# InfiniteNightmare/HNSW-Slim

Measured on AMD Instinct MI355X. Metric: QPS @ recall@10>=0.95 (SIFT-1M d=128, k=10), higher is better.
Workload: dtype f32

## Files before the change

hnsw-slim_amd/csrc/capi_search.cpp:

```cpp
#include "capi_internal.hpp"

#include <cstdio>

static constexpr size_t kMaxLaunchQueries = 32768;

static PlanInput plan_input(const hs_index *ix, size_t k, size_t nq, int mode, bool has_filter, bool want_raw) {
  PlanInput in{};
  const DevIndex &d = ix->dev;
  in.n = ix->info.n; in.dim = ix->info.dim;
  in.has_tile0 = d.tile0 != nullptr; in.has_uptile = d.uptile != nullptr;
  in.maxlevel = d.maxlevel; in.threshold_level = d.threshold_level; in.has_deleted = d.has_deleted; in.kind = d.kind;
  in.ef = ix->ef; in.k = k; in.nq = nq; in.mode = mode;
  in.user_cand_cap = ix->user_cand_cap; in.user_hash_slots = ix->user_hash_slots; in.grow_cand = ix->grow_cand; in.grow_hash = ix->grow_hash;
  in.exact_order = ix->exact_order; in.want_raw = want_raw; in.has_filter = has_filter;
  in.row_fmt = ix->row_fmt; in.f32_resident = ix->f32_resident;
  in.diag = diag();
  return in;
}

static hs_status search_dev_group(hs_index *ix, const float *d_q, size_t nq, size_t k, int mode, uint32_t *l32,
                                  uint64_t *l64, float *dd, uint32_t *cnt, uint32_t *stats, Pair *raw, uint32_t *rawsz,
                                  hipStream_t stream, bool first_group, size_t nq_total, const FilterUse *fu = nullptr) {
  if (!ix) return fail(HS_ERR_INVALID, "null index");
  if (k == 0) return fail(HS_ERR_INVALID, "k must be > 0");
  if (mode != HS_MODE_SLIM_IDS && mode != HS_MODE_PQ) return fail(HS_ERR_INVALID, "bad mode");
  if (ix->info.kind == HS_KIND_SLIMQ) return fail(HS_ERR_INVALID, "SlimQ index: use hs_slimq_search_batch");
  if (mode == HS_MODE_SLIM_IDS && ix->info.kind != HS_KIND_SLIM)
    return fail(HS_ERR_INVALID, "HS_MODE_SLIM_IDS needs a Slim index (searchKnn(q,k,tableint*) exists on HierarchicalNSWSlim only)");
  if (nq > 0x7FFFFFFFu) return fail(HS_ERR_INVALID, "nq too large");
  if (nq == 0) return HS_OK;
  SearchPlan p;
  const char *why = "";
  hs_status ps = plan_search(plan_input(ix, k, nq, mode, fu != nullptr, raw != nullptr), p, &why);
  if (ps != HS_OK) return fail(ps, why);
  HIP_TRY(hipSetDevice(ix->device));
  hs_index::StreamWs *w = ix->stream_ws(stream);
  HIP_TRY(w->status.ensure(nq));
  HIP_TRY(w->spill.ensure(nq * (size_t)p.spill_stride));
  if (w->counters.n < 48) {
    HIP_TRY(w->counters.ensure(48));
    HIP_TRY(hipMemsetAsync(w->counters.p, 0, 48 * sizeof(uint32_t), stream));
  }
  if (first_group) w->last_nq += nq_total;
  if (p.split) {
    HIP_TRY(w->entry.ensure(nq * 4));
    HIP_TRY(w->order.ensure(nq));
  }
  HIP_TRY(w->fb.ensure((size_t)kFbGrid * ((size_t)kFbCand * 2 + kFbSpill)));
  ix->last_kernel = p.name;

  SearchArgs a{};
  FilterArgs fa{};
  if (fu) fa = FilterArgs{fu->fs->bits.p, fu->d_of_query, w->counters.p + 12, (uint32_t)fu->fs->row_words, (uint32_t)fu->fs->nf};
  const FilterArgs *fap = fu ? &fa : nullptr;
  a.queries = d_q; a.nq = (uint32_t)nq; a.k = (uint32_t)k; a.ef = p.ef;
  a.mode = mode; a.mark_ep = (int32_t)p.mark_ep;
  a.out_labels32 = l32; a.out_labels64 = l64; a.out_dists = dd; a.out_counts = cnt; a.stats = stats;
  a.raw_top = raw; a.raw_size = rawsz; a.raw_stride = p.ef;
  a.status = w->status.p;
  a.spill = w->spill.p; a.spill_slots = kSpillSlots; a.spill_stride = p.spill_stride; a.cand2_cap = kCand2Cap;
  a.log_cap = p.log_cap; a.hop_cap = p.hop_cap;
  a.flat = p.flat;
  a.cand_cap = p.cand_cap; a.hash_slots = p.hash_slots; a.vis_bits = p.vis_bits; a.hash_fill_shift = p.hash_fill_shift;
  if (p.family == HS_PLAN_FLAT) { a.fl_nb = p.fl_nb; a.fl_mul = p.fl_mul; a.fl_sh = p.fl_sh; }
  a.counters = w->counters.p; a.pass_id = 0;
  a.select_mask = 1u << ST_TODO; a.grid = (uint32_t)nq;
  auto strict_go = [&](int rows) {
    return rows != ROWS_F32 ? launch_strict_narrow(ix->dev, a, ix->narrow.p, rows, stream, fap) : launch_strict(ix->dev, a, stream, fap);
  };
  auto pass0 = [&]() {
    switch (p.family) {
      case HS_PLAN_FLAT: return p.rows != ROWS_F32 ? launch_flatk_narrow(ix->dev, a, ix->narrow.p, p.rows, stream) : launch_flatk(ix->dev, a, stream);
      case HS_PLAN_LEAN: return launch_lean(ix->dev, a, stream);
      case HS_PLAN_FAST: return p.rows != ROWS_F32 ? launch_fast_narrow(ix->dev, a, ix->narrow.p, p.rows, stream, fap) : launch_fast(ix->dev, a, stream, fap);
      default: return strict_go(p.rows);
    }
  };
  if (p.split) {
    a.entry = reinterpret_cast<uint4 *>(w->entry.p); a.order = w->order.p;
    a.phase = 1;
    HIP_TRY(pass0());
    if (p.skip_order) a.order = nullptr;
    else HIP_TRY(launch_order(a.entry, w->order.p, (uint32_t)nq, stream));
    a.phase = 2;
    HIP_TRY(pass0());
    a.phase = 0;
  } else {
    HIP_TRY(pass0());
  }
  a.select_mask = p.rerun_select_mask; a.grid = (uint32_t)std::min<size_t>(nq, kFbGrid);
  a.cand_cap = p.rerun_cand_cap; a.hash_slots = p.rerun_hash_slots; a.vis_bits = 0; a.hash_fill_shift = 0;
  a.fb_cand = w->fb.p; a.fb_spill = w->fb.p + (size_t)kFbGrid * kFbCand * 2; a.spill_slots = kFbSpill;
  a.counters = w->counters.p + 8; a.pass_id = 2;
  HIP_TRY(strict_go(p.rerun_rows));
  return HS_OK;
}

hs_status search_dev(hs_index *ix, const float *d_q, size_t nq, size_t k, int mode, uint32_t *l32, uint64_t *l64, float *dd,
                     uint32_t *cnt, uint32_t *stats, Pair *raw, uint32_t *rawsz, hipStream_t stream, const FilterUse *fu) {
  if (!ix) return fail(HS_ERR_INVALID, "null index");
  if (nq > 0x7FFFFFFFu) return fail(HS_ERR_INVALID, "nq too large");
  const size_t dim = ix->info.dim, ef = std::max(ix->ef, k);
  for (size_t off = 0; off < nq || off == 0; off += kMaxLaunchQueries) {
    const size_t m = std::min(kMaxLaunchQueries, nq - off);
    const FilterUse g{fu ? fu->fs : nullptr, fu ? fu->d_of_query + off : nullptr};
    hs_status s = search_dev_group(ix, d_q + off * dim, m, k, mode, l32 ? l32 + off * k : nullptr, l64 ? l64 + off * k : nullptr,
                                   dd ? dd + off * k : nullptr, cnt ? cnt + off : nullptr, stats ? stats + off * 4 : nullptr,
                                   raw ? raw + off * ef : nullptr, rawsz ? rawsz + off : nullptr, stream, off == 0, nq, fu ? &g : nullptr);
    if (s != HS_OK || nq == 0) return s;
  }
  return HS_OK;
}

hs_status hs_search_check(hs_index *ix, void *stream) {
  if (!ix) return fail(HS_ERR_INVALID, "null index");
  uint32_t c[13];
  HIP_TRY(hipSetDevice(ix->device));
  hs_index::StreamWs *w = ix->stream_ws((hipStream_t)stream);
  if (!w->counters.p) return HS_OK;
  HIP_TRY(hipMemcpyAsync(c, w->counters.p, sizeof(c), hipMemcpyDeviceToHost, (hipStream_t)stream));
  HIP_TRY(hipMemsetAsync(w->counters.p, 0, sizeof(c), (hipStream_t)stream));
  HIP_TRY(hipStreamSynchronize((hipStream_t)stream));
  const size_t nq = std::max<size_t>(w->last_nq, 1);
  w->last_nq = 0;
  if (diag().verbose) fprintf(stderr, "[hs check] nq %zu: visited overflow %u, candidate overflow %u, tie replays %u, visited-set spills %u | pass 2: %u %u | grow_hash %u grow_cand %u\n",
                       nq, c[0], c[1], c[2], c[3], c[8], c[9], ix->grow_hash, ix->grow_cand);
  if ((size_t)c[3] * 10 > nq && ix->grow_hash < 8 && !ix->user_hash_slots) ix->grow_hash++;
  if ((size_t)(c[1] + c[5]) * 100 > nq && ix->grow_cand < 4 && !ix->user_cand_cap) ix->grow_cand++;
  if (c[12] > 0)
    return fail(HS_ERR_INVALID, std::to_string(c[12]) + " queries named a filter index outside the filter set (count 0 returned for them)");
  if (ix->info.kind == HS_KIND_SLIMQ) {
    if (c[8] > 0) return fail(HS_ERR_CAPACITY, std::to_string(c[8]) + " queries expanded more nodes than the 64 KiB on-chip set holds");
    return HS_OK;
  }
  if (c[8] + c[9] > 0)
    return fail(HS_ERR_CAPACITY, std::to_string(c[8] + c[9]) + " queries exhausted even a whole CU's on-chip scratch");
  return HS_OK;
}

hs_status hs_debug_search_plan(const hs_plan_in *in, hs_plan_out *out) {
  if (!in || !out) return fail(HS_ERR_INVALID, "null argument");
  const char *why = "";
  hs_status s = plan_search(*in, *out, &why);
  return s == HS_OK ? s : fail(s, why);
}
hs_status hs_debug_plan_input(const hs_index *ix, size_t k, size_t nq, int has_filter, int want_raw, hs_plan_in *in) {
  if (!ix || !in) return fail(HS_ERR_INVALID, "null argument");
  *in = plan_input(ix, k, nq, HS_MODE_PQ, has_filter != 0, want_raw != 0);
  return HS_OK;
}

hs_status hs_debug_heap_ops(const uint32_t *ops, size_t n_ops, int wave_pop, uint32_t lds_slots, uint32_t *out_heap, uint32_t *out_pops,
                            uint32_t *out_n) {
  if (!ops || !out_heap || !out_pops || !out_n) return fail(HS_ERR_INVALID, "null argument");
  if (lds_slots < 2 || lds_slots > 8192 || (lds_slots & 1)) return fail(HS_ERR_INVALID, "lds_slots: even, 2..8192");
  DevBuf<uint32_t> d_ops, d_n;
  DevBuf<uint2> d_spill, d_heap, d_pops;
  HIP_TRY(d_ops.alloc(std::max<size_t>(3 * n_ops, 1)));
  HIP_TRY(d_n.alloc(2));
  HIP_TRY(d_spill.alloc(n_ops + 2));
  HIP_TRY(d_heap.alloc(n_ops + 2));
  HIP_TRY(d_pops.alloc(n_ops + 2));
  HIP_TRY(hipMemcpy(d_ops.p, ops, 3 * n_ops * sizeof(uint32_t), hipMemcpyHostToDevice));
  HIP_TRY(flat_heap_ops(d_ops.p, (uint32_t)n_ops, d_spill.p, d_heap.p, d_pops.p, d_n.p, wave_pop, lds_slots, nullptr));
// ... 162 lines not shown
```

hnsw-slim_amd/csrc/engine.hpp:

```cpp
#pragma once
#include <hip/hip_runtime.h>

#include <cstdint>

#include "heap_emul.hpp"

namespace hs {

struct DevIndex {
  const float *vec;
  const uint32_t *row_ptr0;
  const uint32_t *cols;
  const uint32_t *up_base;
  const uint32_t *up_ptr;
  const uint32_t *tile0;
  const uint2 *uptile;
  const uint64_t *labels;
  const uint8_t *deleted;
  uint32_t n, dim, tile_stride, up_stride, ep_base;
  int32_t maxlevel, threshold_level;
  uint32_t enterpoint;
  int32_t has_deleted, kind, metric;
};

enum : uint32_t { ST_TODO = 0, ST_DONE = 1, ST_OVERFLOW = 2, ST_HAZARD = 3 };

struct SearchArgs {
  const float *queries;
  uint32_t nq, k, ef;
  uint32_t cand_cap;
  uint32_t hash_slots;
  uint32_t *spill;
  uint32_t spill_slots, spill_stride, cand2_cap, log_cap;
  int32_t mode;
  int32_t mark_ep;
  uint32_t select_mask;
  uint32_t grid;
  uint32_t *out_labels32;
  uint64_t *out_labels64;
  float *out_dists;
  uint32_t *out_counts;
  uint32_t *stats;
  Pair *raw_top;
  uint32_t *raw_size;
  uint32_t raw_stride;
  uint32_t *status;
  uint32_t *counters;
  uint32_t pass_id;
  uint32_t hash_fill_shift;
  uint32_t flat;
  uint32_t hop_cap;
  uint32_t vis_bits;
  uint32_t phase;
  uint4 *entry;
  const uint32_t *order;
  void *fb_cand;
  uint32_t *fb_spill;
  uint32_t fl_nb, fl_mul, fl_sh;
};

struct FilterArgs {
  const uint32_t *rows;
  const uint32_t *of_query;
  uint32_t *bad;
  uint32_t stride, nf;
};

size_t strict_lds_bytes(uint32_t dim, uint32_t ef, uint32_t cand_cap, uint32_t hash_slots);
size_t fast_lds_bytes(uint32_t dim, uint32_t ef, uint32_t cand_cap, uint32_t hash_slots);
bool fast_supported(const DevIndex &ix, uint32_t ef, uint32_t k, bool has_filter = false);

hipError_t launch_strict(const DevIndex &ix, const SearchArgs &a, hipStream_t stream, const FilterArgs *f = nullptr);
hipError_t launch_order(const uint4 *entry, uint32_t *order, uint32_t nq, hipStream_t stream);
bool lean_supported(const DevIndex &ix, uint32_t ef, uint32_t k);
size_t lean_lds_bytes(uint32_t dim, uint32_t ef, uint32_t cand_cap, uint32_t hash_slots);
hipError_t launch_lean(const DevIndex &ix, const SearchArgs &a, hipStream_t stream);
bool flatk_supported(const DevIndex &ix, uint32_t ef, uint32_t k);
size_t flatk_lds_bytes(uint32_t dim, uint32_t ef, uint32_t nb);
uint32_t flatk_waves_per_cu(uint32_t dim, uint32_t ef);
hipError_t launch_flatk(const DevIndex &ix, const SearchArgs &a, hipStream_t stream);
hipError_t flat_heap_ops(const uint32_t *d_ops, uint32_t n_ops, uint2 *d_spill, uint2 *d_heap, uint2 *d_pops, uint32_t *d_n, int wave_pop,
                         uint32_t lds_slots, hipStream_t stream);
hipError_t launch_fast(const DevIndex &ix, const SearchArgs &a, hipStream_t stream, const FilterArgs *f = nullptr);
hipError_t launch_flatk_narrow(const DevIndex &ix, const SearchArgs &a, const void *rows, int fmt, hipStream_t stream);
hipError_t launch_strict_narrow(const DevIndex &ix, const SearchArgs &a, const void *rows, int fmt, hipStream_t stream, const FilterArgs *f = nullptr);
hipError_t launch_fast_narrow(const DevIndex &ix, const SearchArgs &a, const void *rows, int fmt, hipStream_t stream, const FilterArgs *f = nullptr);
hipError_t launch_narrow_convert(const float *d_vec, void *d_out, int fmt, uint32_t row0, uint32_t nrows, uint32_t dim, uint32_t *d_first_bad,
                                 hipStream_t stream);
hipError_t launch_narrow_widen(const void *d_rows, float *d_vec, int fmt, uint32_t row0, uint32_t nrows, uint32_t dim, hipStream_t stream);
hipError_t launch_filter_pack(const uint8_t *d_allowed, uint32_t *d_words, uint32_t n, uint32_t count, uint32_t row_words, hipStream_t stream);
hipError_t launch_filter_unpack(const uint32_t *d_row, uint8_t *d_allowed, uint32_t n, hipStream_t stream);

}
```

hnsw-slim_amd/csrc/flat_search.hip:

```cpp
#include <hip/hip_runtime.h>

#include <algorithm>
#include <cfloat>
#include <climits>

#include "dist_recipe.hpp"
#include "engine.hpp"
#include "heap_emul.hpp"
#include "narrow_load.hpp"
#include "search_common.hpp"
#include "sorted_insert.hpp"
#include "wave_util.hpp"

namespace hs {

typedef __attribute__((address_space(3))) unsigned char lds_u8;
typedef __attribute__((address_space(3))) uint32_t lds_u32;
typedef __attribute__((address_space(3))) unsigned short lds_u16;
typedef uint32_t hs_u4 __attribute__((ext_vector_type(4)));
typedef __attribute__((address_space(3))) hs_u4 lds_u128;
typedef __attribute__((address_space(3))) float lds_f32;
typedef __attribute__((address_space(3))) hs_f2 lds_f2;
typedef unsigned short hs_us2 __attribute__((ext_vector_type(2)));

static constexpr uint32_t kFlatOvfCap = 64;
static constexpr uint32_t kFlatBucketTags = 7;

struct FlatLds { uint32_t off_q, off_vis, off_ovf, off_nid, total; };
__host__ __device__ inline FlatLds flat_layout(uint32_t dim, uint32_t ef, uint32_t nb) {
  FlatLds l;
  l.off_q = 0;
  l.off_vis = align_up(dim * 4, 16);
  const uint32_t vis_bytes = nb * 16 > (ef + 1) * 8 ? nb * 16 : (ef + 1) * 8;
  l.off_ovf = l.off_vis + align_up(vis_bytes, 16);
  l.off_nid = l.off_ovf + kFlatOvfCap * 4;
  l.total = l.off_nid + 64 * 4;
  return l;
}

__device__ __forceinline__ uint32_t pk_min_u16(uint32_t a, uint32_t b) {
  return __builtin_bit_cast(uint32_t, __builtin_elementwise_min(__builtin_bit_cast(hs_us2, a), __builtin_bit_cast(hs_us2, b)));
}
template <int METRIC>
__device__ __forceinline__ int dkey(float d) {
  const int b = (int)__float_as_uint(d);
  return METRIC == METRIC_L2 ? b : (b ^ ((b >> 31) & 0x7FFFFFFF));
}
template <int METRIC>
__device__ __forceinline__ float key_dist(int k) {
  return __uint_as_float((uint32_t)(METRIC == METRIC_L2 ? k : (k ^ ((k >> 31) & 0x7FFFFFFF))));
}
static constexpr int kFKeyInf = 0x7F800000;
static constexpr uint32_t kFDone = 0x80000000u;

__device__ __forceinline__ int wave_min_i32_f(int v) {
#define HS_SHR_MINI(ctrl) v = min(v, __builtin_amdgcn_update_dpp(INT_MAX, v, ctrl, 0xf, 0xf, false))
  HS_SHR_MINI(0x111); HS_SHR_MINI(0x112); HS_SHR_MINI(0x114); HS_SHR_MINI(0x118);
#undef HS_SHR_MINI
  const int r0 = __builtin_amdgcn_readlane(v, 15), r1 = __builtin_amdgcn_readlane(v, 31);
  const int r2 = __builtin_amdgcn_readlane(v, 47), r3 = __builtin_amdgcn_readlane(v, 63);
  return min(min(r0, r1), min(r2, r3));
}

__host__ __device__ constexpr int flat_row_buffer(int d16) {
#ifdef HS_FLAT_LONG_B
  return d16 <= 0 ? 1 : d16 <= 8 ? d16 : (d16 < HS_FLAT_LONG_B ? d16 : HS_FLAT_LONG_B);
#else
  return d16 <= 0 ? 1 : d16 <= 8 ? d16 : d16 % 30 == 0 ? 30 : d16 % 32 == 0 ? 32 : d16 % 24 == 0 ? 24 : 16;
#endif
}
__host__ __device__ constexpr int flat_waves(int s, int d16) {
#ifdef HS_FLAT_WAVES
  return HS_FLAT_WAVES;
#else
#ifdef HS_FLAT_LONG_WAVES
  return d16 > 8 ? HS_FLAT_LONG_WAVES : d16 < 0 ? 3 : s > 4 ? 4 : 5;
#else
  return d16 > 8 ? 2 : d16 < 0 ? 3 : s > 4 ? 4 : 5;
#endif
#endif
}


template <int METRIC, int D16, typename ROW>
__device__ __forceinline__ float flat_dist8(const ROW *vec, uint32_t dim, const lds_u8 *qv, uint32_t rowid, int s) {
  const lds_f2 *qq = reinterpret_cast<const lds_f2 *>(qv) + s;
  hs_f2 acc = {0.f, 0.f};
  auto step = [&](const hs_f2 q2, const hs_f2 x) {
    if (METRIC == METRIC_L2) {
      const hs_f2 t = q2 - x;
      const hs_f2 p = t * t;
      acc = acc + p;
    } else {
      acc = __builtin_elementwise_fma(q2, x, acc);
    }
  };
  if constexpr (RowKind<ROW>::narrow) {
    const ROW *chunk = vec + (size_t)rowid * dim + (uint32_t)s * (dim >> 3);
    if constexpr (D16 > 0) {
      constexpr int NDW = D16 * (int)sizeof(ROW) / 2;
      static_assert(D16 * sizeof(ROW) % 2 == 0, "a lane's chunk is a whole number of dwords");
      const uint32_t *cp = reinterpret_cast<const uint32_t *>(chunk);
      uint32_t dw[NDW];
#pragma unroll
      for (int j = 0; j + 4 <= NDW; j += 4) {
        const hs_u4_a4 v = *reinterpret_cast<const hs_u4_a4 *>(cp + j);
        dw[j] = v.x; dw[j + 1] = v.y; dw[j + 2] = v.z; dw[j + 3] = v.w;
      }
      if constexpr ((NDW & 2) != 0) {
        const hs_u2_a4 v = *reinterpret_cast<const hs_u2_a4 *>(cp + (NDW & ~3));
        dw[NDW & ~3] = v.x; dw[(NDW & ~3) + 1] = v.y;
      }
      if constexpr ((NDW & 1) != 0) dw[NDW - 1] = cp[NDW - 1];
#pragma unroll
      for (int i = 0; i < D16; i++) {
        if (D16 > 8 && i % 8 == 0) __builtin_amdgcn_sched_barrier(0);
        step(qq[i * 8], narrow_pair((const ROW *)nullptr, dw, i));
      }
    } else {
      constexpr uint32_t RB = D16 == 0 ? 8u : 16u;
      const uint32_t steps = dim >> 4;
      for (uint32_t r0 = 0; r0 < steps; r0 += RB) {
        const uint32_t nb = min(RB, steps - r0);
        hs_f2 buf[RB];
#pragma unroll
        for (uint32_t i = 0; i < RB; i++)
          if (i < nb) buf[i] = narrow_pair_at(chunk, r0 + i);
#pragma unroll
        for (uint32_t i = 0; i < RB; i++)
          if (i < nb) step(qq[(r0 + i) * 8], buf[i]);
      }
    }
  } else {
  const hs_f2 *row = reinterpret_cast<const hs_f2 *>(vec + (size_t)rowid * dim) + s;
  if (D16 > 0) {
    constexpr int B = flat_row_buffer(D16);
    constexpr int R = (D16 > 0 ? D16 : 1) / B, T = (D16 > 0 ? D16 : 1) % B;
    hs_f2 buf[B];
#pragma unroll
    for (int i = 0; i < B; i++) buf[i] = row[i * 8];
#pragma unroll
    for (int i = 0; i < B; i++) {
      if (B > 8 && i % 8 == 0) __builtin_amdgcn_sched_barrier(0);
      step(qq[i * 8], buf[i]);
    }
#pragma unroll 1
    for (int r = 1; r < R; r++) {
#pragma unroll
      for (int i = 0; i < B; i++) buf[i] = row[(r * B + i) * 8];
#pragma unroll
      for (int i = 0; i < B; i++) step(qq[(r * B + i) * 8], buf[i]);
    }
    if (T > 0) {
#pragma unroll
      for (int i = 0; i < T; i++) buf[i] = row[(R * B + i) * 8];
#pragma unroll
      for (int i = 0; i < T; i++) step(qq[(R * B + i) * 8], buf[i]);
    }
  } else {
    constexpr uint32_t RB = D16 == 0 ? 8u : 16u;
    const uint32_t steps = dim >> 4;
    for (uint32_t r0 = 0; r0 < steps; r0 += RB) {
      const uint32_t nb = min(RB, steps - r0);
      hs_f2 buf[RB];
#pragma unroll
      for (uint32_t i = 0; i < RB; i++)
        if (i < nb) buf[i] = row[(r0 + i) * 8];
#pragma unroll
      for (uint32_t i = 0; i < RB; i++)
        if (i < nb) step(qq[(r0 + i) * 8], buf[i]);
    }
  }
  }
  if (METRIC == METRIC_L2) {
    float r = acc.x + acc.y;
#pragma unroll
    for (int k = 1; k < 8; k++) {
      float t;
      asm("s_nop 1\n\tv_add_f32_dpp %0, %1, %2 row_shr:1 row_mask:0xf bank_mask:0xf" : "=v"(t) : "v"(r), "v"(acc.x));
      r = t + acc.y;
    }
    return r;
  } else {
    float hx = acc.x + dpp_f<0x104>(acc.x), hy = acc.y + dpp_f<0x104>(acc.y);
    hx = hx + dpp_f<0x102>(hx); hy = hy + dpp_f<0x102>(hy);
    hx = hx + dpp_f<0x101>(hx); hy = hy + dpp_f<0x101>(hy);
    return 1.0f - (hx + hy);
  }
}

struct FlatHeap {
  lds_u8 *lds;
  uint2 *glob;
  uint32_t L;
};
typedef uint32_t hs_u2 __attribute__((ext_vector_type(2)));
typedef __attribute__((address_space(3))) hs_u2 lds_u64;
template <bool T2>
__device__ __forceinline__ uint2 fh_get(const FlatHeap &h, uint32_t s) {
  if (!T2 || s < h.L) { const hs_u2 v = *reinterpret_cast<lds_u64 *>(h.lds + s * 8); return make_uint2(v.x, v.y); }
  return h.glob[s];
}
template <bool T2>
__device__ __forceinline__ void fh_set(const FlatHeap &h, uint32_t s, uint2 v) {
  if (!T2 || s < h.L) *reinterpret_cast<lds_u64 *>(h.lds + s * 8) = hs_u2{v.x, v.y};
  else h.glob[s] = v;
}
template <bool T2>
__device__ __forceinline__ uint4 fh_get2(const FlatHeap &h, uint32_t s ) {
  if (!T2 || s < h.L) { const hs_u4 v = *reinterpret_cast<lds_u128 *>(h.lds + s * 8); return make_uint4(v.x, v.y, v.z, v.w); }
  return *reinterpret_cast<const uint4 *>(&h.glob[s]);
}
template <bool T2>
__device__ __forceinline__ void fh_push(const FlatHeap &h, uint32_t n , float d, uint32_t id, int lane) {
  const uint32_t anc = n >> (lane + 1);
  const bool has = anc != 0 && lane < 31;
  uint2 p = make_uint2(0, 0);
  if (has) p = fh_get<T2>(h, anc);
  const unsigned long long rises = hs_ballot(has && __uint_as_float(p.x) > d);
  const uint32_t r = __ffsll((long long)~rises) - 1;
  if ((uint32_t)lane < r) fh_set<T2>(h, n >> lane, p);
  if ((uint32_t)lane == r) fh_set<T2>(h, n >> r, make_uint2(__float_as_uint(d), id));
}
template <bool T2>
__device__ __forceinline__ void fh_pop(const FlatHeap &h, uint32_t n ) {
  if (n <= 1) return;
  const uint2 v = fh_get<T2>(h, n);
  const uint32_t len = n - 1;
  uint32_t hole = 0, child = 0;
  while (child < (len - 1) / 2) {
    child = 2 * (child + 1);
    const uint4 two = fh_get2<T2>(h, child);
    const bool left = __uint_as_float(two.z) > __uint_as_float(two.x);
    fh_set<T2>(h, hole + 1, left ? make_uint2(two.x, two.y) : make_uint2(two.z, two.w));
    child = left ? child - 1 : child;
    hole = child;
  }
  if ((len & 1) == 0 && child == (len - 2) / 2) {
    child = 2 * (child + 1);
    fh_set<T2>(h, hole + 1, fh_get<T2>(h, child));
    hole = child - 1;
  }
  const float vd = __uint_as_float(v.x);
  while (hole > 0) {
    const uint32_t parent = (hole - 1) >> 1;
    const uint2 p = fh_get<T2>(h, parent + 1);
    if (!(__uint_as_float(p.x) > vd)) break;
    fh_set<T2>(h, hole + 1, p);
    hole = parent;
  }
  fh_set<T2>(h, hole + 1, v);
}

__device__ __forceinline__ void fh_pop_wave(const FlatHeap &h, uint32_t n , int lane) {
  if (n <= 1) return;
  const uint2 v = fh_get<false>(h, n);
  const uint32_t len = n - 1;
  uint32_t hole = 0;
  const uint32_t dl = lane < 1 ? 0u : (lane < 3 ? 1u : 2u);
  const uint32_t ol = (uint32_t)lane + 1u - (1u << dl);
  while (true) {
    const uint32_t node = ((hole + 1u) << dl) - 1u + ol;
    const bool two = lane < 7 && 2u * node + 2u < len;
    uint4 pr = make_uint4(0, 0, 0, 0);
    if (two) pr = fh_get2<false>(h, 2u * node + 2u);
    const bool right = !(__uint_as_float(pr.z) > __uint_as_float(pr.x));
    const unsigned long long vm = hs_ballot(two), rm = hs_ballot(two && right);
    uint32_t l = 0, path = 0, last = 0;
    bool open = true;
#pragma unroll
    for (int kk = 0; kk < 3; kk++) {
      const bool ok = open && ((vm >> l) & 1ull);
// ... 778 lines not shown
```

hnsw-slim_amd/csrc/search_plan.cpp:

```cpp
#include "search_plan.hpp"

#include <algorithm>
#include <cstdlib>
#include <cstring>

#include "engine.hpp"

namespace hs {

Diag diag_from_env() {
  Diag d{};
  const char *kernel = getenv("HS_KERNEL");
  d.kernel = kernel && !strcmp(kernel, "lean") ? HS_PLAN_KERNEL_LEAN : kernel && !strcmp(kernel, "fast") ? HS_PLAN_KERNEL_FAST : HS_PLAN_KERNEL_DEFAULT;
  const char *lean = getenv("HS_LEAN_MIN_EF");
  d.lean_forced = lean != nullptr;
  d.lean_min_ef = lean ? (uint32_t)atoi(lean) : kLeanMinEf;
  d.order = getenv("HS_ORDER") ? atoi(getenv("HS_ORDER")) : -1;
  d.flat = !(getenv("HS_FLAT") && atoi(getenv("HS_FLAT")) == 0);
  d.vis16 = !(getenv("HS_VIS16") && atoi(getenv("HS_VIS16")) == 0);
  d.flat_waves_per_cu = getenv("HS_FLAT_WAVES_PER_CU") ? atoi(getenv("HS_FLAT_WAVES_PER_CU")) : 0;
  const char *zc = getenv("HS_ZERO_COPY");
  d.zero_copy = zc && !strcmp(zc, "0") ? HS_PLAN_ZERO_COPY_OFF : zc && !strcmp(zc, "in") ? HS_PLAN_ZERO_COPY_IN : HS_PLAN_ZERO_COPY_ON;
  d.verbose = getenv("HS_VERBOSE") != nullptr;
  const char *fused = getenv("HS_SLIMQ_FUSED");
  d.slimq_fused = !(fused && fused[0] == '0');
  return d;
}
const Diag &diag() {
  static const Diag d = diag_from_env();
  return d;
}

const char *kernel_name(int family, int rows) {
  static const char *const names[4][3] = {
      {"hs::flat_kernel", "hs::flat_kernel_f16", "hs::flat_kernel_u8"},
      {"hs::lean_kernel", "hs::lean_kernel", "hs::lean_kernel"},
      {"hs::fast_kernel", "hs::fast_kernel_f16", "hs::fast_kernel_u8"},
      {"hs::strict_kernel", "hs::strict_kernel_f16", "hs::strict_kernel_u8"},
  };
  return names[family][rows];
}

namespace {

struct Shape {
  uint32_t ef, cand_cap, cand_cap_fast, hash_slots;
  uint32_t q_hash_slots, q_bits;
  uint32_t l_cand_cap, l_hash_slots;
  uint32_t fb_cand_cap, fb_hash_slots;
};
uint32_t log_cap_for(uint32_t ef) { return ef <= 256 ? kLogCap : 2 * kLogCap; }
uint32_t hop_cap_for(uint32_t ef) { return ef <= 256 ? kHopCap : 4 * kHopCap; }
uint32_t spill_stride_for(uint32_t ef) { return kSpillSlots + 2 * kCand2Cap + 2 * log_cap_for(ef) + hop_cap_for(ef) / 4 + kParkWords; }

hs_status plan_shape(const PlanInput &in, Shape &s, const char **msg) {
  const size_t ef = std::max<size_t>(in.ef, in.k);
  if (ef > (1u << 20)) { *msg = "ef too large"; return HS_ERR_INVALID; }
  s.ef = (uint32_t)ef;
  s.cand_cap_fast = in.user_cand_cap ? in.user_cand_cap : (uint32_t)(4.4 * ef + 64);
  s.cand_cap_fast = (s.cand_cap_fast + 1) & ~1u;
  s.cand_cap = in.user_cand_cap ? in.user_cand_cap : (uint32_t)((3 * ef + 256) << in.grow_cand);
  s.cand_cap = (s.cand_cap + 1) & ~1u;
  const uint32_t want = (uint32_t)((450 + 5 * ef) * (1.0 + 0.25 * in.grow_hash) / 0.75);
  s.hash_slots = in.user_hash_slots ? (in.user_hash_slots + 63) / 64 * 64 : (want + 63) / 64 * 64;
  {
    const uint32_t n_vis = in.user_hash_slots ? in.user_hash_slots : (uint32_t)((450 + 5 * ef) * (1.0 + 0.25 * in.grow_hash));
    uint32_t nb = 4;
    while (nb * 5.0 < n_vis && nb < (1u << 14)) nb <<= 1;
    uint32_t bbits = 0, idbits = 1;
    while ((1u << bbits) < nb) bbits++;
    while (idbits < 32 && ((uint64_t)1 << idbits) < (uint64_t)std::max<size_t>(in.n, 2)) idbits++;
    const uint32_t B = std::max(idbits, bbits);
    s.q_hash_slots = nb * 4;
    s.q_bits = (in.diag.vis16 && B - bbits <= 16 && B < 32) ? B : 0;
  }
  const uint32_t dim = (uint32_t)in.dim;
  {
    uint32_t lc = in.user_cand_cap ? in.user_cand_cap : (uint32_t)((2.5 * ef + 130) * (1u << in.grow_cand));
    s.l_cand_cap = std::max<uint32_t>((lc + 1) & ~1u, 16);
    const uint32_t lh = in.user_hash_slots ? in.user_hash_slots : (uint32_t)((520 + 5 * ef) * (1.0 + 0.25 * in.grow_hash) / 0.875);
    s.l_hash_slots = (lh + 63) / 64 * 64;
  }
  while (strict_lds_bytes(dim, s.ef, s.cand_cap, s.hash_slots) > kLdsPerCU && s.hash_slots > 256) s.hash_slots >>= 1;
  while (strict_lds_bytes(dim, s.ef, s.cand_cap, s.hash_slots) > kLdsPerCU && s.cand_cap > 128) s.cand_cap = (s.cand_cap / 2 + 1) & ~1u;
  if (strict_lds_bytes(dim, s.ef, s.cand_cap, s.hash_slots) > kLdsPerCU) {
    *msg = "ef/dim do not fit the 160 KiB LDS of one CU";
    return HS_ERR_CAPACITY;
  }
  s.fb_cand_cap = kFbCand;
  s.fb_hash_slots = kFbHash;
  while (strict_lds_bytes(dim, s.ef, 0, s.fb_hash_slots) > kLdsPerCU && s.fb_hash_slots > 256) s.fb_hash_slots >>= 1;
  return HS_OK;
}

struct FlatPlan { uint32_t nb, mul, sh, vis_bits; bool ok; };
FlatPlan plan_flat(const PlanInput &in, uint32_t ef) {
  FlatPlan f{};
  const uint32_t dim = (uint32_t)in.dim;
  uint32_t idbits = 1;
  while (idbits < 32 && ((uint64_t)1 << idbits) < (uint64_t)std::max<size_t>(in.n, 2)) idbits++;
  f.vis_bits = idbits;
  uint32_t nb = in.user_hash_slots ? std::max<uint32_t>(in.user_hash_slots / 4, 8) : (uint32_t)((450 + 5.0 * ef) * (1.0 + 0.25 * in.grow_hash) / 3.2);
  nb = std::max<uint32_t>(nb, 8);
  if (!in.user_hash_slots) {
    const size_t total = flatk_lds_bytes(dim, ef, nb);
    const size_t env_waves = (size_t)in.diag.flat_waves_per_cu;
    const size_t max_waves = env_waves ? env_waves : flatk_waves_per_cu(dim, ef);
    size_t waves = std::min<size_t>(max_waves, kLdsPerCU / std::max<size_t>(total, 1));
    if (waves >= 1) {
      const size_t share = std::min<size_t>((kLdsPerCU / waves) & ~size_t(15), 64 * 1024);
      if (share > total) nb += (uint32_t)((share - total) / 16);
    }
  }
// ... 92 lines not shown
```

hnsw-slim_amd/csrc/search_plan.hpp:

```cpp
#pragma once
#include <cstddef>
#include <cstdint>

#include "../../include/hnsw_slim_amd.h"

#pragma GCC visibility push(hidden)
namespace hs {

using Diag = hs_plan_diag;
Diag diag_from_env();
const Diag &diag();

using PlanInput = hs_plan_in;
using SearchPlan = hs_plan_out;

static constexpr size_t kLdsPerCU = 160 * 1024;
static constexpr uint32_t kFbGrid = 32, kFbCand = 32768, kFbSpill = 131072, kFbHash = 2048;
static constexpr uint32_t kLeanMinEf = 64;
static constexpr uint32_t kSpillSlots = 8192;
static constexpr uint32_t kCand2Cap = 4096;
static constexpr uint32_t kLogCap = 4096;
static constexpr uint32_t kHopCap = 4096;
static constexpr uint32_t kParkWords = 2048;
static constexpr size_t kOrderMinQueries = 6144;
inline bool split_launch(const Diag &d, size_t nq) { return d.order < 0 ? nq >= kOrderMinQueries : d.order != 0; }

const char *kernel_name(int family, int rows);

hs_status plan_search(const PlanInput &in, SearchPlan &out, const char **msg);

}
#pragma GCC visibility pop
```

Baseline: 15.04 million.

## Run upper-layer HNSW descent in a dedicated lightweight kernel for flat plans

For split launches with the flat kernel family, the phase-1 greedy descent through the upper HNSW levels now runs in a separate 64-thread kernel with small LDS and high waves-per-EU, instead of the heavy flat search kernel. It prefetches neighbour tiles for candidates ahead and stages them in LDS. The aim is to avoid the flat kernel's large LDS and register footprint limiting occupancy during the cheap descent phase. It adds a kernel launch and a new code path, and the old behaviour can be restored with HS_DESCENT=flat. The shared distance helpers move into a common header.

```diff
diff --git a/hnsw-slim_amd/csrc/capi_search.cpp b/hnsw-slim_amd/csrc/capi_search.cpp
--- a/hnsw-slim_amd/csrc/capi_search.cpp
+++ b/hnsw-slim_amd/csrc/capi_search.cpp
@@ -79,7 +79,8 @@
   if (p.split) {
     a.entry = reinterpret_cast<uint4 *>(w->entry.p); a.order = w->order.p;
     a.phase = 1;
-    HIP_TRY(pass0());
+    if (p.family == HS_PLAN_FLAT && !descent_in_flat_kernel()) HIP_TRY(launch_flat_descent(ix->dev, a, ix->narrow.p, p.rows, stream));
+    else HIP_TRY(pass0());
     if (p.skip_order) a.order = nullptr;
     else HIP_TRY(launch_order(a.entry, w->order.p, (uint32_t)nq, stream));
     a.phase = 2;
diff --git a/hnsw-slim_amd/csrc/descent_search.hip b/hnsw-slim_amd/csrc/descent_search.hip
--- /dev/null
+++ b/hnsw-slim_amd/csrc/descent_search.hip
@@ -0,0 +1,197 @@
+#include <hip/hip_runtime.h>
+
+#include <algorithm>
+#include <climits>
+
+#include "engine.hpp"
+#include "flat_dist.hpp"
+#include "narrow_load.hpp"
+#include "narrow_rows.hpp"
+#include "search_common.hpp"
+#include "wave_util.hpp"
+
+namespace hs {
+
+typedef uint32_t hs_u2 __attribute__((ext_vector_type(2)));
+typedef __attribute__((address_space(3))) hs_u2 lds_u64;
+
+static constexpr uint32_t kDescentAhead = 256;
+static constexpr uint32_t kDescentStage = 64;
+
+__host__ __device__ inline uint32_t descent_stage_off(uint32_t dim) { return align_up(dim * 4, 16); }
+__host__ __device__ inline uint32_t descent_lds(uint32_t dim) { return descent_stage_off(dim) + kDescentStage * 8; }
+
+__host__ __device__ constexpr int descent_waves(int d16) { return d16 > 8 ? 2 : d16 < 0 ? 7 : 8; }
+
+template <int METRIC, int D16, typename ROW>
+__device__ __forceinline__ void descend_one(const DevIndex &ix, const SearchArgs &a, const uint32_t qi, lds_u8 *smem, const ROW *rows) {
+  auto fresh_lane = []() -> uint32_t { uint32_t l = threadIdx.x; asm volatile("" : "+v"(l)); return l; };
+  const int lane = (int)fresh_lane();
+  constexpr int OWN = METRIC == METRIC_L2 ? 7 : 0;
+  const uint32_t dim = D16 > 0 ? (uint32_t)D16 * 16u : ix.dim;
+  lds_u8 *qv = smem;
+  lds_u64 *stage = reinterpret_cast<lds_u64 *>(smem + descent_stage_off(dim));
+  const uint32_t us = ix.up_stride;
+  const uint32_t u16 = us >> 4;
+  const uint32_t cmul = u16 == 3 ? 86u : 256u >> (u16 >> 1);
+  const uint2 none = make_uint2(kNone, kNone);
+  auto tile = [&](uint32_t slot, uint32_t at) -> uint2 { return ix.uptile[(size_t)slot * us + at]; };
+  auto ahead_cand = [&](int t, uint32_t ln) -> uint32_t { return (((uint32_t)t * 4u + (ln >> 4)) * cmul) >> 8; };
+  auto ahead_off = [&](int t, uint32_t ln, uint32_t c) -> uint32_t { return (((uint32_t)t * 4u + (ln >> 4) - c * u16) << 4) | (ln & 15u); };
+
+  for (uint32_t i = lane; i < dim; i += 64) reinterpret_cast<lds_f32 *>(qv)[i] = a.queries[(size_t)qi * dim + i];
+  wave_sync();
+
+  uint32_t n_dist = 1, n_hops = 0;
+  uint32_t cur = ix.enterpoint, cur_b = ix.ep_base;
+  uint2 pr = none;
+  if (ix.maxlevel > 0 && cur_b != kNone && (uint32_t)lane < us) pr = tile(cur_b + (uint32_t)ix.maxlevel - 1u, lane);
+  float curdist;
+  {
+    const float d = flat_dist8<METRIC, D16>(rows, dim, qv, cur, lane & 7);
+    curdist = __uint_as_float(__builtin_amdgcn_readlane(__float_as_uint(d), OWN));
+  }
+  for (int lvl = ix.maxlevel; lvl > 0; lvl--) {
+    uint2 dn = none;
+    while (true) {
+      n_hops++;
+      if (cur_b == kNone) break;
+      const uint32_t ln = fresh_lane();
+      const int s8 = (int)(ln & 7u);
+      const uint32_t grp = ln >> 3;
+      const uint32_t m = __popcll(hs_ballot(pr.x != kNone));
+      if (lvl >= 2 && ln < us) dn = tile(cur_b + (uint32_t)lvl - 2u, ln);
+      if (m == 0) break;
+      n_dist += m;
+      const bool ahead = m * us <= kDescentAhead;
+      uint2 ct[4];
+      uint32_t cb[4];
+#pragma unroll
+      for (int t = 0; t < 4; t++) {
+        const uint32_t c = ahead_cand(t, ln), b = __shfl(pr.y, (int)c, 64);
+        cb[t] = (ahead && c < m) ? b : kNone;
+      }
+#pragma unroll
+      for (int t = 0; t < 4; t++) {
+        ct[t] = none;
+        if (cb[t] != kNone) ct[t] = tile(cb[t] + (uint32_t)lvl - 1u, ahead_off(t, ln, ahead_cand(t, ln)));
+      }
+      int best_key = INT_MAX;
+      uint32_t best_at = 0;
+      for (uint32_t base = 0; base < m; base += 8) {
+        const uint32_t j = base + grp;
+        const uint32_t rid = __shfl(pr.x, (int)(j < m ? j : base), 64);
+        const float d = flat_dist8<METRIC, D16>(rows, dim, qv, rid, s8);
+        const int ky = (s8 == OWN && j < m) ? dkey<METRIC>(d) : INT_MAX;
+        const int mn = wave_min_i32_f(ky);
+        if (mn < best_key) {
+          best_key = mn;
+          best_at = base + ((uint32_t)(__ffsll((long long)hs_ballot(ky == mn)) - 1) >> 3);
+        }
+      }
+      if (!(best_key < dkey<METRIC>(curdist))) break;
+      curdist = key_dist<METRIC>(best_key);
+      cur = __builtin_amdgcn_readlane(pr.x, best_at);
+      cur_b = __builtin_amdgcn_readlane(pr.y, best_at);
+      if (cur_b == kNone) continue;
+      const uint32_t l2 = fresh_lane();
+      if (ahead) {
+#pragma unroll
+        for (int t = 0; t < 4; t++) {
+          const uint32_t c = ahead_cand(t, l2);
+          if (c == best_at) stage[ahead_off(t, l2, c)] = hs_u2{ct[t].x, ct[t].y};
+        }
+        wave_sync();
+        pr = none;
+        if (l2 < us) { const hs_u2 v = stage[l2]; pr = make_uint2(v.x, v.y); }
+        wave_sync();
+      } else {
+        pr = none;
+        if (l2 < us) pr = tile(cur_b + (uint32_t)lvl - 1u, l2);
+      }
+    }
+    pr = dn;
+  }
+  if (lane == 0) a.entry[qi] = make_uint4(cur, __float_as_uint(curdist), n_dist, n_hops);
+}
+
+#define HS_DESCENT_KERNEL_BODY(ROWS)                                                                                     \
+  extern __shared__ __align__(16) unsigned char smem_raw[];                                                              \
+  lds_u8 *smem = (lds_u8 *)smem_raw;                                                                                     \
+  for (uint32_t qi = blockIdx.x; qi < a.nq; qi += gridDim.x) {                                                           \
+    descend_one<METRIC, D16>(ix, a, qi, smem, ROWS);                                                                     \
+    wave_sync();                                                                                                         \
+  }
+#if !defined(HS_TU_ROWS) || HS_TU_ROWS == 0
+template <int METRIC, int D16>
+__global__ void __launch_bounds__(64) __attribute__((amdgpu_waves_per_eu(descent_waves(D16)))) descent_kernel(DevIndex ix, SearchArgs a) {
+  HS_DESCENT_KERNEL_BODY(ix.vec)
+}
+#define HS_DESCENT_KERNEL descent_kernel
+#define HS_DESCENT_ROWS_ARG
+#elif HS_TU_ROWS == 1
+template <int METRIC, int D16>
+__global__ void __launch_bounds__(64) __attribute__((amdgpu_waves_per_eu(descent_waves(D16)))) descent_kernel_u8(DevIndex ix, SearchArgs a, const uint8_t *rows) {
+  HS_DESCENT_KERNEL_BODY(rows)
+}
+#define HS_DESCENT_KERNEL descent_kernel_u8
+#define HS_DESCENT_ROWS_ARG , reinterpret_cast<const uint8_t *>(rows)
+#else
+template <int METRIC, int D16>
+__global__ void __launch_bounds__(64) __attribute__((amdgpu_waves_per_eu(descent_waves(D16)))) descent_kernel_f16(DevIndex ix, SearchArgs a, const _Float16 *rows) {
+  HS_DESCENT_KERNEL_BODY(rows)
+}
+#define HS_DESCENT_KERNEL descent_kernel_f16
+#define HS_DESCENT_ROWS_ARG , reinterpret_cast<const _Float16 *>(rows)
+#endif
+
+template <int METRIC, int D16>
+static hipError_t descent_launch_d(const DevIndex &ix, const SearchArgs &a, const void *rows, hipStream_t stream) {
+  if (a.nq == 0) return hipSuccess;
+  const size_t lds = descent_lds(ix.dim);
+  if (lds > 64 * 1024) {
+    hipError_t e = hipFuncSetAttribute(reinterpret_cast<const void *>(HS_DESCENT_KERNEL<METRIC, D16>), hipFuncAttributeMaxDynamicSharedMemorySize, (int)lds);
+    if (e != hipSuccess) return e;
+  }
+  hipLaunchKernelGGL((HS_DESCENT_KERNEL<METRIC, D16>), dim3(std::max(1u, std::min(a.grid, a.nq))), dim3(64), lds, stream, ix, a HS_DESCENT_ROWS_ARG);
+  return hipGetLastError();
+}
+template <int METRIC>
+static hipError_t descent_launch_s(const DevIndex &ix, const SearchArgs &a, const void *rows, hipStream_t stream) {
+  if (ix.dim == 128) return descent_launch_d<METRIC, 8>(ix, a, rows, stream);
+  if (ix.dim == 96) return descent_launch_d<METRIC, 6>(ix, a, rows, stream);
+  if (ix.dim == 960) return descent_launch_d<METRIC, 60>(ix, a, rows, stream);
+  if (ix.dim > 256) return descent_launch_d<METRIC, -1>(ix, a, rows, stream);
+  return descent_launch_d<METRIC, 0>(ix, a, rows, stream);
+}
+
+#if !defined(HS_TU_ROWS) || HS_TU_ROWS == 0
+#define HS_DESCENT_LAUNCHER(metric) launch_descent_f32_##metric
+#elif HS_TU_ROWS == 1
+#define HS_DESCENT_LAUNCHER(metric) launch_descent_u8_##metric
+#else
+#define HS_DESCENT_LAUNCHER(metric) launch_descent_f16_##metric
+#endif
+#if !defined(HS_TU_METRIC) || HS_TU_METRIC == 0
+hipError_t HS_DESCENT_LAUNCHER(l2)(const DevIndex &ix, const SearchArgs &a, const void *rows, hipStream_t stream) { return descent_launch_s<METRIC_L2>(ix, a, rows, stream); }
+#endif
+#if !defined(HS_TU_METRIC) || HS_TU_METRIC == 1
+hipError_t HS_DESCENT_LAUNCHER(ip)(const DevIndex &ix, const SearchArgs &a, const void *rows, hipStream_t stream) { return descent_launch_s<METRIC_IP>(ix, a, rows, stream); }
+#endif
+
+#if (!defined(HS_TU_ROWS) || HS_TU_ROWS == 0) && (!defined(HS_TU_METRIC) || HS_TU_METRIC == 0)
+hipError_t launch_descent_f32_ip(const DevIndex &ix, const SearchArgs &a, const void *rows, hipStream_t stream);
+hipError_t launch_descent_u8_l2(const DevIndex &ix, const SearchArgs &a, const void *rows, hipStream_t stream);
+hipError_t launch_descent_u8_ip(const DevIndex &ix, const SearchArgs &a, const void *rows, hipStream_t stream);
+hipError_t launch_descent_f16_l2(const DevIndex &ix, const SearchArgs &a, const void *rows, hipStream_t stream);
+hipError_t launch_descent_f16_ip(const DevIndex &ix, const SearchArgs &a, const void *rows, hipStream_t stream);
+hipError_t launch_flat_descent(const DevIndex &ix, const SearchArgs &a, const void *narrow_rows, int row_fmt, hipStream_t stream) {
+  const bool l2 = ix.metric == METRIC_L2;
+  if (row_fmt == ROWS_U8) return l2 ? launch_descent_u8_l2(ix, a, narrow_rows, stream) : launch_descent_u8_ip(ix, a, narrow_rows, stream);
+  if (row_fmt == ROWS_F16) return l2 ? launch_descent_f16_l2(ix, a, narrow_rows, stream) : launch_descent_f16_ip(ix, a, narrow_rows, stream);
+  if (ix.vec == nullptr && ix.n > 0) return hipErrorInvalidDevicePointer;
+  return l2 ? launch_descent_f32_l2(ix, a, nullptr, stream) : launch_descent_f32_ip(ix, a, nullptr, stream);
+}
+#endif
+
+}
diff --git a/hnsw-slim_amd/csrc/descent_search_f16.hip b/hnsw-slim_amd/csrc/descent_search_f16.hip
--- /dev/null
+++ b/hnsw-slim_amd/csrc/descent_search_f16.hip
@@ -0,0 +1,2 @@
+#define HS_TU_ROWS 2
+#include "descent_search.hip"
diff --git a/hnsw-slim_amd/csrc/descent_search_u8.hip b/hnsw-slim_amd/csrc/descent_search_u8.hip
--- /dev/null
+++ b/hnsw-slim_amd/csrc/descent_search_u8.hip
@@ -0,0 +1,2 @@
+#define HS_TU_ROWS 1
+#include "descent_search.hip"
diff --git a/hnsw-slim_amd/csrc/engine.hpp b/hnsw-slim_amd/csrc/engine.hpp
--- a/hnsw-slim_amd/csrc/engine.hpp
+++ b/hnsw-slim_amd/csrc/engine.hpp
@@ -79,6 +79,7 @@
 size_t flatk_lds_bytes(uint32_t dim, uint32_t ef, uint32_t nb);
 uint32_t flatk_waves_per_cu(uint32_t dim, uint32_t ef);
 hipError_t launch_flatk(const DevIndex &ix, const SearchArgs &a, hipStream_t stream);
+hipError_t launch_flat_descent(const DevIndex &ix, const SearchArgs &a, const void *narrow_rows, int row_fmt, hipStream_t stream);
 hipError_t flat_heap_ops(const uint32_t *d_ops, uint32_t n_ops, uint2 *d_spill, uint2 *d_heap, uint2 *d_pops, uint32_t *d_n, int wave_pop,
                          uint32_t lds_slots, hipStream_t stream);
 hipError_t launch_fast(const DevIndex &ix, const SearchArgs &a, hipStream_t stream, const FilterArgs *f = nullptr);
diff --git a/hnsw-slim_amd/csrc/flat_dist.hpp b/hnsw-slim_amd/csrc/flat_dist.hpp
--- /dev/null
+++ b/hnsw-slim_amd/csrc/flat_dist.hpp
@@ -0,0 +1,152 @@
+#pragma once
+#include <hip/hip_runtime.h>
+
+#include <climits>
+#include <cstdint>
+
+#include "dist_recipe.hpp"
+#include "narrow_load.hpp"
+#include "wave_util.hpp"
+
+namespace hs {
+
+typedef __attribute__((address_space(3))) unsigned char lds_u8;
+typedef __attribute__((address_space(3))) float lds_f32;
+typedef __attribute__((address_space(3))) hs_f2 lds_f2;
+
+template <int METRIC>
+__device__ __forceinline__ int dkey(float d) {
+  const int b = (int)__float_as_uint(d);
+  return METRIC == METRIC_L2 ? b : (b ^ ((b >> 31) & 0x7FFFFFFF));
+}
+template <int METRIC>
+__device__ __forceinline__ float key_dist(int k) {
+  return __uint_as_float((uint32_t)(METRIC == METRIC_L2 ? k : (k ^ ((k >> 31) & 0x7FFFFFFF))));
+}
+
+__device__ __forceinline__ int wave_min_i32_f(int v) {
+#define HS_SHR_MINI(ctrl) v = min(v, __builtin_amdgcn_update_dpp(INT_MAX, v, ctrl, 0xf, 0xf, false))
+  HS_SHR_MINI(0x111); HS_SHR_MINI(0x112); HS_SHR_MINI(0x114); HS_SHR_MINI(0x118);
+#undef HS_SHR_MINI
+  const int r0 = __builtin_amdgcn_readlane(v, 15), r1 = __builtin_amdgcn_readlane(v, 31);
+  const int r2 = __builtin_amdgcn_readlane(v, 47), r3 = __builtin_amdgcn_readlane(v, 63);
+  return min(min(r0, r1), min(r2, r3));
+}
+
+__host__ __device__ constexpr int flat_row_buffer(int d16) {
+#ifdef HS_FLAT_LONG_B
+  return d16 <= 0 ? 1 : d16 <= 8 ? d16 : (d16 < HS_FLAT_LONG_B ? d16 : HS_FLAT_LONG_B);
+#else
+  return d16 <= 0 ? 1 : d16 <= 8 ? d16 : d16 % 30 == 0 ? 30 : d16 % 32 == 0 ? 32 : d16 % 24 == 0 ? 24 : 16;
+#endif
+}
+
+
+template <int METRIC, int D16, typename ROW>
+__device__ __forceinline__ float flat_dist8(const ROW *vec, uint32_t dim, const lds_u8 *qv, uint32_t rowid, int s) {
+  const lds_f2 *qq = reinterpret_cast<const lds_f2 *>(qv) + s;
+  hs_f2 acc = {0.f, 0.f};
+  auto step = [&](const hs_f2 q2, const hs_f2 x) {
+    if (METRIC == METRIC_L2) {
+      const hs_f2 t = q2 - x;
+      const hs_f2 p = t * t;
+      acc = acc + p;
+    } else {
+      acc = __builtin_elementwise_fma(q2, x, acc);
+    }
+  };
+  if constexpr (RowKind<ROW>::narrow) {
+    const ROW *chunk = vec + (size_t)rowid * dim + (uint32_t)s * (dim >> 3);
+    if constexpr (D16 > 0) {
+      constexpr int NDW = D16 * (int)sizeof(ROW) / 2;
+      static_assert(D16 * sizeof(ROW) % 2 == 0, "a lane's chunk is a whole number of dwords");
+      const uint32_t *cp = reinterpret_cast<const uint32_t *>(chunk);
+      uint32_t dw[NDW];
+#pragma unroll
+      for (int j = 0; j + 4 <= NDW; j += 4) {
+        const hs_u4_a4 v = *reinterpret_cast<const hs_u4_a4 *>(cp + j);
+        dw[j] = v.x; dw[j + 1] = v.y; dw[j + 2] = v.z; dw[j + 3] = v.w;
+      }
+      if constexpr ((NDW & 2) != 0) {
+        const hs_u2_a4 v = *reinterpret_cast<const hs_u2_a4 *>(cp + (NDW & ~3));
+        dw[NDW & ~3] = v.x; dw[(NDW & ~3) + 1] = v.y;
+      }
+      if constexpr ((NDW & 1) != 0) dw[NDW - 1] = cp[NDW - 1];
+#pragma unroll
+      for (int i = 0; i < D16; i++) {
+        if (D16 > 8 && i % 8 == 0) __builtin_amdgcn_sched_barrier(0);
+        step(qq[i * 8], narrow_pair((const ROW *)nullptr, dw, i));
+      }
+    } else {
+      constexpr uint32_t RB = D16 == 0 ? 8u : 16u;
+      const uint32_t steps = dim >> 4;
+      for (uint32_t r0 = 0; r0 < steps; r0 += RB) {
+        const uint32_t nb = min(RB, steps - r0);
+        hs_f2 buf[RB];
+#pragma unroll
+        for (uint32_t i = 0; i < RB; i++)
+          if (i < nb) buf[i] = narrow_pair_at(chunk, r0 + i);
+#pragma unroll
+        for (uint32_t i = 0; i < RB; i++)
+          if (i < nb) step(qq[(r0 + i) * 8], buf[i]);
+      }
+    }
+  } else {
+  const hs_f2 *row = reinterpret_cast<const hs_f2 *>(vec + (size_t)rowid * dim) + s;
+  if (D16 > 0) {
+    constexpr int B = flat_row_buffer(D16);
+    constexpr int R = (D16 > 0 ? D16 : 1) / B, T = (D16 > 0 ? D16 : 1) % B;
+    hs_f2 buf[B];
+#pragma unroll
+    for (int i = 0; i < B; i++) buf[i] = row[i * 8];
+#pragma unroll
+    for (int i = 0; i < B; i++) {
+      if (B > 8 && i % 8 == 0) __builtin_amdgcn_sched_barrier(0);
+      step(qq[i * 8], buf[i]);
+    }
+#pragma unroll 1
+    for (int r = 1; r < R; r++) {
+#pragma unroll
+      for (int i = 0; i < B; i++) buf[i] = row[(r * B + i) * 8];
+#pragma unroll
+      for (int i = 0; i < B; i++) step(qq[(r * B + i) * 8], buf[i]);
+    }
+    if (T > 0) {
+#pragma unroll
+      for (int i = 0; i < T; i++) buf[i] = row[(R * B + i) * 8];
+#pragma unroll
+      for (int i = 0; i < T; i++) step(qq[(R * B + i) * 8], buf[i]);
+    }
+  } else {
+    constexpr uint32_t RB = D16 == 0 ? 8u : 16u;
+    const uint32_t steps = dim >> 4;
+    for (uint32_t r0 = 0; r0 < steps; r0 += RB) {
+      const uint32_t nb = min(RB, steps - r0);
+      hs_f2 buf[RB];
+#pragma unroll
+      for (uint32_t i = 0; i < RB; i++)
+        if (i < nb) buf[i] = row[(r0 + i) * 8];
+#pragma unroll
+      for (uint32_t i = 0; i < RB; i++)
+        if (i < nb) step(qq[(r0 + i) * 8], buf[i]);
+    }
+  }
+  }
+  if (METRIC == METRIC_L2) {
+    float r = acc.x + acc.y;
+#pragma unroll
+    for (int k = 1; k < 8; k++) {
+      float t;
+      asm("s_nop 1\n\tv_add_f32_dpp %0, %1, %2 row_shr:1 row_mask:0xf bank_mask:0xf" : "=v"(t) : "v"(r), "v"(acc.x));
+      r = t + acc.y;
+    }
+    return r;
+  } else {
+    float hx = acc.x + dpp_f<0x104>(acc.x), hy = acc.y + dpp_f<0x104>(acc.y);
+    hx = hx + dpp_f<0x102>(hx); hy = hy + dpp_f<0x102>(hy);
+    hx = hx + dpp_f<0x101>(hx); hy = hy + dpp_f<0x101>(hy);
+    return 1.0f - (hx + hy);
+  }
+}
+
+}
diff --git a/hnsw-slim_amd/csrc/flat_search.hip b/hnsw-slim_amd/csrc/flat_search.hip
--- a/hnsw-slim_amd/csrc/flat_search.hip
+++ b/hnsw-slim_amd/csrc/flat_search.hip
@@ -6,6 +6,7 @@
 
 #include "dist_recipe.hpp"
 #include "engine.hpp"
+#include "flat_dist.hpp"
 #include "heap_emul.hpp"
 #include "narrow_load.hpp"
 #include "search_common.hpp"
@@ -14,13 +15,10 @@
 
 namespace hs {
 
-typedef __attribute__((address_space(3))) unsigned char lds_u8;
 typedef __attribute__((address_space(3))) uint32_t lds_u32;
 typedef __attribute__((address_space(3))) unsigned short lds_u16;
 typedef uint32_t hs_u4 __attribute__((ext_vector_type(4)));
 typedef __attribute__((address_space(3))) hs_u4 lds_u128;
-typedef __attribute__((address_space(3))) float lds_f32;
-typedef __attribute__((address_space(3))) hs_f2 lds_f2;
 typedef unsigned short hs_us2 __attribute__((ext_vector_type(2)));
 
 static constexpr uint32_t kFlatOvfCap = 64;
@@ -41,34 +39,9 @@
 __device__ __forceinline__ uint32_t pk_min_u16(uint32_t a, uint32_t b) {
   return __builtin_bit_cast(uint32_t, __builtin_elementwise_min(__builtin_bit_cast(hs_us2, a), __builtin_bit_cast(hs_us2, b)));
 }
-template <int METRIC>
-__device__ __forceinline__ int dkey(float d) {
-  const int b = (int)__float_as_uint(d);
-  return METRIC == METRIC_L2 ? b : (b ^ ((b >> 31) & 0x7FFFFFFF));
-}
-template <int METRIC>
-__device__ __forceinline__ float key_dist(int k) {
-  return __uint_as_float((uint32_t)(METRIC == METRIC_L2 ? k : (k ^ ((k >> 31) & 0x7FFFFFFF))));
-}
 static constexpr int kFKeyInf = 0x7F800000;
 static constexpr uint32_t kFDone = 0x80000000u;
 
-__device__ __forceinline__ int wave_min_i32_f(int v) {
-#define HS_SHR_MINI(ctrl) v = min(v, __builtin_amdgcn_update_dpp(INT_MAX, v, ctrl, 0xf, 0xf, false))
-  HS_SHR_MINI(0x111); HS_SHR_MINI(0x112); HS_SHR_MINI(0x114); HS_SHR_MINI(0x118);
-#undef HS_SHR_MINI
-  const int r0 = __builtin_amdgcn_readlane(v, 15), r1 = __builtin_amdgcn_readlane(v, 31);
-  const int r2 = __builtin_amdgcn_readlane(v, 47), r3 = __builtin_amdgcn_readlane(v, 63);
-  return min(min(r0, r1), min(r2, r3));
-}
-
-__host__ __device__ constexpr int flat_row_buffer(int d16) {
-#ifdef HS_FLAT_LONG_B
-  return d16 <= 0 ? 1 : d16 <= 8 ? d16 : (d16 < HS_FLAT_LONG_B ? d16 : HS_FLAT_LONG_B);
-#else
-  return d16 <= 0 ? 1 : d16 <= 8 ? d16 : d16 % 30 == 0 ? 30 : d16 % 32 == 0 ? 32 : d16 % 24 == 0 ? 24 : 16;
-#endif
-}
 __host__ __device__ constexpr int flat_waves(int s, int d16) {
 #ifdef HS_FLAT_WAVES
   return HS_FLAT_WAVES;
@@ -81,113 +54,6 @@
 #endif
 }
 
-
-template <int METRIC, int D16, typename ROW>
-__device__ __forceinline__ float flat_dist8(const ROW *vec, uint32_t dim, const lds_u8 *qv, uint32_t rowid, int s) {
-  const lds_f2 *qq = reinterpret_cast<const lds_f2 *>(qv) + s;
-  hs_f2 acc = {0.f, 0.f};
-  auto step = [&](const hs_f2 q2, const hs_f2 x) {
-    if (METRIC == METRIC_L2) {
-      const hs_f2 t = q2 - x;
-      const hs_f2 p = t * t;
-      acc = acc + p;
-    } else {
-      acc = __builtin_elementwise_fma(q2, x, acc);
-    }
-  };
-  if constexpr (RowKind<ROW>::narrow) {
-    const ROW *chunk = vec + (size_t)rowid * dim + (uint32_t)s * (dim >> 3);
-    if constexpr (D16 > 0) {
-      constexpr int NDW = D16 * (int)sizeof(ROW) / 2;
-      static_assert(D16 * sizeof(ROW) % 2 == 0, "a lane's chunk is a whole number of dwords");
-      const uint32_t *cp = reinterpret_cast<const uint32_t *>(chunk);
-      uint32_t dw[NDW];
-#pragma unroll
-      for (int j = 0; j + 4 <= NDW; j += 4) {
-        const hs_u4_a4 v = *reinterpret_cast<const hs_u4_a4 *>(cp + j);
-        dw[j] = v.x; dw[j + 1] = v.y; dw[j + 2] = v.z; dw[j + 3] = v.w;
-      }
-      if constexpr ((NDW & 2) != 0) {
-        const hs_u2_a4 v = *reinterpret_cast<const hs_u2_a4 *>(cp + (NDW & ~3));
-        dw[NDW & ~3] = v.x; dw[(NDW & ~3) + 1] = v.y;
-      }
-      if constexpr ((NDW & 1) != 0) dw[NDW - 1] = cp[NDW - 1];
-#pragma unroll
-      for (int i = 0; i < D16; i++) {
-        if (D16 > 8 && i % 8 == 0) __builtin_amdgcn_sched_barrier(0);
-        step(qq[i * 8], narrow_pair((const ROW *)nullptr, dw, i));
-      }
-    } else {
-      constexpr uint32_t RB = D16 == 0 ? 8u : 16u;
-      const uint32_t steps = dim >> 4;
-      for (uint32_t r0 = 0; r0 < steps; r0 += RB) {
-        const uint32_t nb = min(RB, steps - r0);
-        hs_f2 buf[RB];
-#pragma unroll
-        for (uint32_t i = 0; i < RB; i++)
-          if (i < nb) buf[i] = narrow_pair_at(chunk, r0 + i);
-#pragma unroll
-        for (uint32_t i = 0; i < RB; i++)
-          if (i < nb) step(qq[(r0 + i) * 8], buf[i]);
-      }
-    }
-  } else {
-  const hs_f2 *row = reinterpret_cast<const hs_f2 *>(vec + (size_t)rowid * dim) + s;
-  if (D16 > 0) {
-    constexpr int B = flat_row_buffer(D16);
-    constexpr int R = (D16 > 0 ? D16 : 1) / B, T = (D16 > 0 ? D16 : 1) % B;
-    hs_f2 buf[B];
-#pragma unroll
-    for (int i = 0; i < B; i++) buf[i] = row[i * 8];
-#pragma unroll
-    for (int i = 0; i < B; i++) {
-      if (B > 8 && i % 8 == 0) __builtin_amdgcn_sched_barrier(0);
-      step(qq[i * 8], buf[i]);
-    }
-#pragma unroll 1
-    for (int r = 1; r < R; r++) {
-#pragma unroll
-      for (int i = 0; i < B; i++) buf[i] = row[(r * B + i) * 8];
-#pragma unroll
-      for (int i = 0; i < B; i++) step(qq[(r * B + i) * 8], buf[i]);
-    }
-    if (T > 0) {
-#pragma unroll
-      for (int i = 0; i < T; i++) buf[i] = row[(R * B + i) * 8];
-#pragma unroll
-      for (int i = 0; i < T; i++) step(qq[(R * B + i) * 8], buf[i]);
-    }
-  } else {
-    constexpr uint32_t RB = D16 == 0 ? 8u : 16u;
-    const uint32_t steps = dim >> 4;
-    for (uint32_t r0 = 0; r0 < steps; r0 += RB) {
-      const uint32_t nb = min(RB, steps - r0);
-      hs_f2 buf[RB];
-#pragma unroll
-      for (uint32_t i = 0; i < RB; i++)
-        if (i < nb) buf[i] = row[(r0 + i) * 8];
-#pragma unroll
-      for (uint32_t i = 0; i < RB; i++)
-        if (i < nb) step(qq[(r0 + i) * 8], buf[i]);
-    }
-  }
-  }
-  if (METRIC == METRIC_L2) {
-    float r = acc.x + acc.y;
-#pragma unroll
-    for (int k = 1; k < 8; k++) {
-      float t;
-      asm("s_nop 1\n\tv_add_f32_dpp %0, %1, %2 row_shr:1 row_mask:0xf bank_mask:0xf" : "=v"(t) : "v"(r), "v"(acc.x));
-      r = t + acc.y;
-    }
-    return r;
-  } else {
-    float hx = acc.x + dpp_f<0x104>(acc.x), hy = acc.y + dpp_f<0x104>(acc.y);
-    hx = hx + dpp_f<0x102>(hx); hy = hy + dpp_f<0x102>(hy);
-    hx = hx + dpp_f<0x101>(hx); hy = hy + dpp_f<0x101>(hy);
-    return 1.0f - (hx + hy);
-  }
-}
 
 struct FlatHeap {
   lds_u8 *lds;
diff --git a/hnsw-slim_amd/csrc/search_plan.cpp b/hnsw-slim_amd/csrc/search_plan.cpp
--- a/hnsw-slim_amd/csrc/search_plan.cpp
+++ b/hnsw-slim_amd/csrc/search_plan.cpp
@@ -8,8 +8,12 @@
 
 namespace hs {
 
+static bool g_descent_flat = false;
+
 Diag diag_from_env() {
   Diag d{};
+  const char *descent = getenv("HS_DESCENT");
+  g_descent_flat = descent && !strcmp(descent, "flat");
   const char *kernel = getenv("HS_KERNEL");
   d.kernel = kernel && !strcmp(kernel, "lean") ? HS_PLAN_KERNEL_LEAN : kernel && !strcmp(kernel, "fast") ? HS_PLAN_KERNEL_FAST : HS_PLAN_KERNEL_DEFAULT;
   const char *lean = getenv("HS_LEAN_MIN_EF");
@@ -29,6 +33,10 @@
 const Diag &diag() {
   static const Diag d = diag_from_env();
   return d;
+}
+bool descent_in_flat_kernel() {
+  static const bool flat = (diag(), g_descent_flat);
+  return flat;
 }
 
 const char *kernel_name(int family, int rows) {
diff --git a/hnsw-slim_amd/csrc/search_plan.hpp b/hnsw-slim_amd/csrc/search_plan.hpp
--- a/hnsw-slim_amd/csrc/search_plan.hpp
+++ b/hnsw-slim_amd/csrc/search_plan.hpp
@@ -10,6 +10,7 @@
 using Diag = hs_plan_diag;
 Diag diag_from_env();
 const Diag &diag();
+bool descent_in_flat_kernel();
 
 using PlanInput = hs_plan_in;
 using SearchPlan = hs_plan_out;
```

Result: slower. 14.85 million (-1.3%).
